# MircoWerner/VkRadixSort

Measured on AMD Instinct MI355X. Metric: Gkeys/s sorting 10^8 uint32 at 1/2/4/8 MI355X; % of HBM roofline, higher is better.
Workload: dtype u32

## Files before the change

vkradixsort_amd/csrc/vrs_local_sort.hpp:

```cpp
#pragma once
#include "vrs_device.hpp"

namespace vrs {

constexpr int kLeanRow = 512 + 64;
constexpr int kLeanMaxVec = 7;
template <bool STREAM>
__device__ __forceinline__ void store_sorted(uint4 *p, const uint4 &q) {
    if constexpr (STREAM) {
        typedef uint32_t u32x4 __attribute__((ext_vector_type(4)));
        const u32x4 v = {q.x, q.y, q.z, q.w};
        __builtin_nontemporal_store(v, reinterpret_cast<u32x4 *>(p));
    } else {
        *p = q;
    }
}

template <int STRIDE, int VEC>
__device__ __forceinline__ void load_rows(uint32_t (&k)[4 * VEC], const uint32_t *src, uint32_t words, uint32_t t) {
    const uint32_t nvec = (words + 3u) / 4u;
#pragma unroll
    for (int j = 0; j < VEC; ++j) {
        uint32_t v = j * STRIDE + t;
        if (j == VEC - 1) v = v < nvec ? v : nvec - 1u;
        const uint4 q = reinterpret_cast<const uint4 *>(src)[v];
        k[4 * j] = q.x;
        k[4 * j + 1] = q.y;
        k[4 * j + 2] = q.z;
        k[4 * j + 3] = q.w;
    }
}

template <int THREADS, int VEC, bool GUARD, bool STREAM = false, bool ALIGNED_IN = false>
__device__ __forceinline__ void lean_sort_body(uint32_t (&k)[4 * VEC], uint32_t *abase, uint32_t mis, uint32_t n, uint32_t *s_keys,
                                               uint32_t *s_hist2, uint32_t *s_tmp, bool guard1, bool guard2, uint32_t mis_in) {
    constexpr int WAVES = THREADS / 64, ITEMS = 4 * VEC, PER = 512 / THREADS;
    const uint32_t tid = threadIdx.x, lane = tid & 63u, wave = tid >> 6;
    const uint32_t end = mis + n;
    const uint32_t nvec = (end + 3u) / 4u;
    uint32_t rank[ITEMS];
    uint32_t *s_hist = s_hist2 + WAVES * kLeanRow;
#pragma unroll
    for (int j = 0; j < VEC; ++j)
#pragma unroll
        for (int c = 0; c < 4; ++c) {
            uint32_t a = (k[4 * j + c] << 2) & 0x7FCu;
            if (ALIGNED_IN ? j >= VEC - 2 : (j == 0 || j == VEC - 1)) {
                const uint32_t q = 4u * (j * THREADS + tid) + c;
                a = (q - mis_in < n) ? a : 2048u + 4u * lane;
            }
            uint32_t *counter = reinterpret_cast<uint32_t *>(reinterpret_cast<char *>(s_hist) + a);
            if (GUARD && guard1) {
                const uint32_t a0 = __builtin_amdgcn_readfirstlane(a);
                if (__ballot(a == a0) == ~0ull) {
                    uint32_t old = 0;
                    if (lane == 0u) old = __hip_atomic_fetch_add(counter, 256u, __ATOMIC_RELAXED, __HIP_MEMORY_SCOPE_WORKGROUP);
                    rank[4 * j + c] = __builtin_amdgcn_readfirstlane(old) + 4u * lane;
                    continue;
                }
            }
            rank[4 * j + c] = __hip_atomic_fetch_add(counter, 4u, __ATOMIC_RELAXED, __HIP_MEMORY_SCOPE_WORKGROUP);
        }
    __syncthreads();
    {
        uint32_t c[PER], total = 0;
        if constexpr (PER == 2) {
            const uint2 q = reinterpret_cast<const uint2 *>(s_hist)[tid];
            c[0] = q.x;
            c[1] = q.y;
            total = q.x + q.y;
        } else {
            c[0] = s_hist[tid];
            total = c[0];
        }
        uint32_t incl = total;
#pragma unroll
        for (int o = 1; o < 64; o <<= 1) {
            const uint32_t t = __shfl_up(incl, o);
            if (lane >= static_cast<uint32_t>(o)) incl += t;
        }
        if (lane == 63u) s_tmp[wave] = incl;
        __syncthreads();
        uint32_t acc = incl - total;
#pragma unroll
        for (int v = 0; v < WAVES; ++v) acc += (static_cast<uint32_t>(v) < wave) ? s_tmp[v] : 0u;
        if constexpr (PER == 2) reinterpret_cast<uint2 *>(s_hist)[tid] = make_uint2(acc, acc + c[0]);
        else s_hist[tid] = acc;
    }
    __syncthreads();
#pragma unroll
    for (int j = 0; j < VEC; ++j)
#pragma unroll
        for (int c = 0; c < 4; ++c) {
            uint32_t a = (opaque(k[4 * j + c]) << 2) & 0x7FCu;
            if (ALIGNED_IN ? j >= VEC - 2 : (j == 0 || j == VEC - 1)) {
                const uint32_t q = 4u * (j * THREADS + tid) + c;
                const bool valid = q - mis_in < n;
                a = valid ? a : 2048u + 4u * lane;
                const uint32_t r = rank[4 * j + c] + *reinterpret_cast<const uint32_t *>(reinterpret_cast<const char *>(s_hist) + a);
                rank[4 * j + c] = valid ? r : 4u * (q < mis_in ? n + q : q);
                continue;
            }
            rank[4 * j + c] += *reinterpret_cast<const uint32_t *>(reinterpret_cast<const char *>(s_hist) + a);
        }
#pragma unroll
    for (int i = 0; i < ITEMS; ++i) {
        const uint32_t Lb = rank[i];
        const uint32_t ph = (Lb & ~1023u) | ((Lb & 252u) << 2) | ((Lb >> 6) & 12u);
        *reinterpret_cast<uint32_t *>(reinterpret_cast<char *>(s_keys) + ph) = k[i];
    }
    __syncthreads();
    const uint32_t seg = wave * (ITEMS * 64);
#pragma unroll
    for (int g = 0; g < VEC; ++g) {
        const uint4 t = reinterpret_cast<const uint4 *>(s_keys + seg + g * 256)[lane];
        k[4 * g] = t.x;
        k[4 * g + 1] = t.y;
        k[4 * g + 2] = t.z;
        k[4 * g + 3] = t.w;
    }
    char *my = reinterpret_cast<char *>(s_hist2 + wave * kLeanRow);
    constexpr int kEmptyItems = (4 * THREADS + 3 + 63) / 64;
    constexpr int kFirstMaybeEmpty = ITEMS >= kEmptyItems ? ITEMS - kEmptyItems : 0;
#pragma unroll
    for (int i = 0; i < ITEMS; ++i) {
        uint32_t a = (k[i] >> 7) & 0x7FCu;
        if (i >= kFirstMaybeEmpty) a = (seg + i * 64 + lane < n) ? a : 2048u + 4u * lane;
        uint32_t *counter = reinterpret_cast<uint32_t *>(my + a);
        if (GUARD && guard2) {
            const uint32_t a0 = __builtin_amdgcn_readfirstlane(a);
            if (__ballot(a == a0) == ~0ull) {
                uint32_t old = 0;
                if (lane == 0u) old = __hip_atomic_fetch_add(counter, 256u, __ATOMIC_RELAXED, __HIP_MEMORY_SCOPE_WORKGROUP);
                rank[i] = __builtin_amdgcn_readfirstlane(old) + 4u * lane;
                continue;
            }
        }
        rank[i] = __hip_atomic_fetch_add(counter, 4u, __ATOMIC_RELAXED, __HIP_MEMORY_SCOPE_WORKGROUP);
    }
    __syncthreads();
    {
        uint32_t c[WAVES][PER], total = 0;
#pragma unroll
        for (int v = 0; v < WAVES; ++v) {
            if constexpr (PER == 2) {
                const uint2 q = reinterpret_cast<const uint2 *>(s_hist2 + v * kLeanRow)[tid];
                c[v][0] = q.x;
                c[v][1] = q.y;
                total += q.x + q.y;
            } else {
                c[v][0] = s_hist2[v * kLeanRow + tid];
                total += c[v][0];
            }
        }
        uint32_t incl = total;
#pragma unroll
        for (int o = 1; o < 64; o <<= 1) {
            const uint32_t t = __shfl_up(incl, o);
            if (lane >= static_cast<uint32_t>(o)) incl += t;
        }
        if (lane == 63u) s_tmp[wave] = incl;
        __syncthreads();
        uint32_t acc = incl - total + 4u * mis;
#pragma unroll
        for (int v = 0; v < WAVES; ++v) acc += (static_cast<uint32_t>(v) < wave) ? s_tmp[v] : 0u;
        uint32_t out[WAVES][PER];
#pragma unroll
        for (int p_ = 0; p_ < PER; ++p_)
#pragma unroll
            for (int v = 0; v < WAVES; ++v) {
                out[v][p_] = acc;
                acc += c[v][p_];
            }
#pragma unroll
        for (int v = 0; v < WAVES; ++v) {
            if constexpr (PER == 2) reinterpret_cast<uint2 *>(s_hist2 + v * kLeanRow)[tid] = make_uint2(out[v][0], out[v][1]);
            else s_hist2[v * kLeanRow + tid] = out[v][0];
        }
    }
    __syncthreads();
#pragma unroll
    for (int i = 0; i < ITEMS; ++i) {
        uint32_t a = (opaque(k[i]) >> 7) & 0x7FCu;
        if (i >= kFirstMaybeEmpty) {
            const uint32_t L = seg + i * 64 + lane;
            a = L < n ? a : 2048u + 4u * lane;
            const uint32_t r = rank[i] + *reinterpret_cast<const uint32_t *>(my + a);
            rank[i] = L < n ? r : 4u * (mis + L);
            continue;
        }
        rank[i] += *reinterpret_cast<const uint32_t *>(my + a);
    }
#pragma unroll
    for (int i = 0; i < ITEMS; ++i) *reinterpret_cast<uint32_t *>(reinterpret_cast<char *>(s_keys) + rank[i]) = k[i];
    __syncthreads();
#pragma unroll
    for (int j = 0; j < VEC; ++j) {
        const uint32_t v = j * THREADS + tid;
        if (j > 0 && j < VEC - 1) {
            store_sorted<STREAM>(reinterpret_cast<uint4 *>(abase) + v, reinterpret_cast<const uint4 *>(s_keys)[v]);
        } else if (v < nvec) {
            const uint4 q4 = reinterpret_cast<const uint4 *>(s_keys)[v];
            const uint32_t q = 4u * v;
            if (q >= mis && q + 4u <= end) {
                store_sorted<STREAM>(reinterpret_cast<uint4 *>(abase) + v, q4);
            } else {
                if (q + 0u - mis < n) abase[q + 0u] = q4.x;
                if (q + 1u - mis < n) abase[q + 1u] = q4.y;
                if (q + 2u - mis < n) abase[q + 2u] = q4.z;
                if (q + 3u - mis < n) abase[q + 3u] = q4.w;
            }
        }
    }
}

__device__ __forceinline__ void wave_phase() {
    __builtin_amdgcn_fence(__ATOMIC_RELEASE, "wavefront");
    __builtin_amdgcn_wave_barrier();
    __builtin_amdgcn_fence(__ATOMIC_ACQUIRE, "wavefront");
}
__device__ __forceinline__ void wave_scan512(uint32_t *tbl, uint32_t lane, uint32_t start) {
    uint4 a = reinterpret_cast<uint4 *>(tbl)[2 * lane], b = reinterpret_cast<uint4 *>(tbl)[2 * lane + 1];
    const uint32_t s = a.x + a.y + a.z + a.w + b.x + b.y + b.z + b.w;
    uint32_t incl = s;
#pragma unroll
    for (int o = 1; o < 64; o <<= 1) {
        const uint32_t t = __shfl_up(incl, o);
        if (lane >= static_cast<uint32_t>(o)) incl += t;
    }
    uint32_t acc = incl - s + start;
    uint4 oa, ob;
    oa.x = acc; acc += a.x; oa.y = acc; acc += a.y; oa.z = acc; acc += a.z; oa.w = acc; acc += a.w;
    ob.x = acc; acc += b.x; ob.y = acc; acc += b.y; ob.z = acc; acc += b.z; ob.w = acc;
    reinterpret_cast<uint4 *>(tbl)[2 * lane] = oa;
    reinterpret_cast<uint4 *>(tbl)[2 * lane + 1] = ob;
}
template <int VEC, bool GUARD, bool STREAM = false, bool ALIGNED_IN = false>
__device__ __forceinline__ void wave_sort_body(uint32_t (&k)[4 * VEC], uint32_t *abase, uint32_t mis, uint32_t n, uint32_t *s_keys,
                                               uint32_t *tbl, bool guard1, bool guard2, uint32_t mis_in) {
    constexpr int ITEMS = 4 * VEC;
    const uint32_t lane = threadIdx.x & 63u;
    const uint32_t end = mis + n, nvec = (end + 3u) / 4u;
    uint32_t rank[ITEMS];
    char *tb = reinterpret_cast<char *>(tbl);
    const auto zero_table = [&] {
        reinterpret_cast<uint4 *>(tbl)[2 * lane] = make_uint4(0, 0, 0, 0);
        reinterpret_cast<uint4 *>(tbl)[2 * lane + 1] = make_uint4(0, 0, 0, 0);
        if (lane < 16u) reinterpret_cast<uint4 *>(tbl)[128 + lane] = make_uint4(0, 0, 0, 0);
    };
    const auto ranked_add = [&](uint32_t a, bool guard) -> uint32_t {
        uint32_t *counter = reinterpret_cast<uint32_t *>(tb + a);
        if (GUARD && guard) {
            const uint32_t a0 = __builtin_amdgcn_readfirstlane(a);
            if (__ballot(a == a0) == ~0ull) {
                uint32_t old = 0;
                if (lane == 0u) old = __hip_atomic_fetch_add(counter, 256u, __ATOMIC_RELAXED, __HIP_MEMORY_SCOPE_WORKGROUP);
                return __builtin_amdgcn_readfirstlane(old) + 4u * lane;
            }
        }
        return __hip_atomic_fetch_add(counter, 4u, __ATOMIC_RELAXED, __HIP_MEMORY_SCOPE_WORKGROUP);
    };
#pragma unroll
    for (int i = 0; i < ITEMS; ++i) {
        uint32_t a = (k[i] << 2) & 0x7FCu;
        if (ALIGNED_IN ? i >= ITEMS - 8 : (i < 4 || i >= ITEMS - 4)) {
            const uint32_t q = 4u * ((i >> 2) * 64 + lane) + (i & 3);
            a = (q - mis_in < n) ? a : 2048u + 4u * lane;
        }
        rank[i] = ranked_add(a, guard1);
    }
    wave_phase();
    wave_scan512(tbl, lane, 0u);
    wave_phase();
#pragma unroll
    for (int i = 0; i < ITEMS; ++i) {
        uint32_t a = (opaque(k[i]) << 2) & 0x7FCu;
        if (ALIGNED_IN ? i >= ITEMS - 8 : (i < 4 || i >= ITEMS - 4)) {
            const uint32_t q = 4u * ((i >> 2) * 64 + lane) + (i & 3);
            const bool valid = q - mis_in < n;
            a = valid ? a : 2048u + 4u * lane;
            const uint32_t r = rank[i] + *reinterpret_cast<const uint32_t *>(tb + a);
            rank[i] = valid ? r : 4u * (q < mis_in ? n + q : q);
            continue;
        }
        rank[i] += *reinterpret_cast<const uint32_t *>(tb + a);
    }
#pragma unroll
    for (int i = 0; i < ITEMS; ++i) {
        const uint32_t Lb = rank[i];
        const uint32_t ph = (Lb & ~1023u) | ((Lb & 252u) << 2) | ((Lb >> 6) & 12u);
        *reinterpret_cast<uint32_t *>(reinterpret_cast<char *>(s_keys) + ph) = k[i];
    }
    wave_phase();
    zero_table();
#pragma unroll
    for (int g = 0; g < VEC; ++g) {
        const uint4 t = reinterpret_cast<const uint4 *>(s_keys + g * 256)[lane];
        k[4 * g] = t.x;
        k[4 * g + 1] = t.y;
        k[4 * g + 2] = t.z;
        k[4 * g + 3] = t.w;
    }
    wave_phase();
#pragma unroll
    for (int i = 0; i < ITEMS; ++i) {
        uint32_t a = (k[i] >> 7) & 0x7FCu;
        a = (i * 64 + lane < n) ? a : 2048u + 4u * lane;
        rank[i] = ranked_add(a, guard2);
    }
    wave_phase();
    wave_scan512(tbl, lane, 4u * mis);
    wave_phase();
#pragma unroll
    for (int i = 0; i < ITEMS; ++i) {
        const uint32_t L = i * 64 + lane;
        uint32_t a = (opaque(k[i]) >> 7) & 0x7FCu;
        a = L < n ? a : 2048u + 4u * lane;
        const uint32_t r = rank[i] + *reinterpret_cast<const uint32_t *>(tb + a);
        rank[i] = L < n ? r : 4u * (mis + L);
    }
#pragma unroll
    for (int i = 0; i < ITEMS; ++i) *reinterpret_cast<uint32_t *>(reinterpret_cast<char *>(s_keys) + rank[i]) = k[i];
    wave_phase();
#pragma unroll
    for (int j = 0; j < VEC; ++j) {
        const uint32_t v = j * 64 + lane;
        if (v < nvec) {
            const uint4 q4 = reinterpret_cast<const uint4 *>(s_keys)[v];
            const uint32_t q = 4u * v;
            if (q >= mis && q + 4u <= end) {
                store_sorted<STREAM>(reinterpret_cast<uint4 *>(abase) + v, q4);
            } else {
                if (q + 0u - mis < n) abase[q + 0u] = q4.x;
                if (q + 1u - mis < n) abase[q + 1u] = q4.y;
                if (q + 2u - mis < n) abase[q + 2u] = q4.z;
                if (q + 3u - mis < n) abase[q + 3u] = q4.w;
            }
        }
    }
}

struct NoHook {
    __device__ __forceinline__ void operator()() const {}
};
template <int THREADS, int ITEMS, int BITS, bool PAIRS, bool STABLE, typename K = uint32_t, typename Hook = NoHook>
__device__ __forceinline__ void local_pass(K (&key)[ITEMS], uint32_t (&val)[PAIRS ? ITEMS : 1], K *s_keys,
                                           uint32_t *s_vals, uint32_t *s_hist, uint32_t *s_tmp, uint32_t shift, uint32_t n, Hook scanned = Hook()) {
    constexpr int WAVES = THREADS / 64, BINS = 1 << BITS, TABLES = STABLE ? WAVES : 1, PER = BINS >= THREADS ? BINS / THREADS : 1;
    static_assert(PER * THREADS == BINS || (PER == 1 && THREADS % BINS == 0), "every scanning thread owns PER whole bins");
    const uint32_t tid = threadIdx.x, lane = tid & 63u, wave = tid >> 6;
    const bool scans = THREADS <= BINS || tid < static_cast<uint32_t>(BINS);
    for (uint32_t c = tid; c < TABLES * BINS; c += THREADS) s_hist[c] = 0;
    __syncthreads();
    uint32_t *my = s_hist + (STABLE ? wave * BINS : 0u);
    const uint32_t seg = wave * (ITEMS * 64) + lane;
    uint32_t rank[ITEMS];
#pragma unroll
    for (int i = 0; i < ITEMS; ++i) {
        rank[i] = seg + i * 64;
        if (rank[i] < n) {
            const uint32_t d = static_cast<uint32_t>(key[i] >> shift) & (BINS - 1);
            const uint32_t d0 = __builtin_amdgcn_readfirstlane(d);
            const uint64_t active = __ballot(1);
            if (__ballot(d == d0) == active) {
                uint32_t old = 0;
                if (__builtin_amdgcn_mbcnt_hi(static_cast<uint32_t>(active >> 32), __builtin_amdgcn_mbcnt_lo(static_cast<uint32_t>(active), 0u)) == 0u)
                    old = __hip_atomic_fetch_add(&my[d0], static_cast<uint32_t>(__popcll(active)), __ATOMIC_RELAXED, __HIP_MEMORY_SCOPE_WORKGROUP);
                rank[i] = __builtin_amdgcn_readfirstlane(old) +
                          __builtin_amdgcn_mbcnt_hi(static_cast<uint32_t>(active >> 32), __builtin_amdgcn_mbcnt_lo(static_cast<uint32_t>(active), 0u));
            } else {
                rank[i] = __hip_atomic_fetch_add(&my[d], 1u, __ATOMIC_RELAXED, __HIP_MEMORY_SCOPE_WORKGROUP);
            }
        }
    }
    __syncthreads();
    {
        uint32_t c[TABLES][PER], total = 0;
#pragma unroll
        for (int v = 0; v < TABLES; ++v) {
            if constexpr (PER == 2) {
                const uint2 q = reinterpret_cast<const uint2 *>(s_hist + v * BINS)[tid];
                c[v][0] = q.x;
                c[v][1] = q.y;
                total += q.x + q.y;
            } else {
#pragma unroll
                for (int p_ = 0; p_ < PER; ++p_) {
                    c[v][p_] = scans ? s_hist[v * BINS + tid * PER + p_] : 0u;
                    total += c[v][p_];
                }
            }
        }
        uint32_t incl = total;
#pragma unroll
        for (int o = 1; o < 64; o <<= 1) {
            const uint32_t t = __shfl_up(incl, o);
            if (lane >= static_cast<uint32_t>(o)) incl += t;
        }
        if (lane == 63u) s_tmp[wave] = incl;
        __syncthreads();
        uint32_t acc = incl - total;
#pragma unroll
        for (int v = 0; v < WAVES; ++v) acc += (static_cast<uint32_t>(v) < wave) ? s_tmp[v] : 0u;
        uint32_t out[TABLES][PER];
#pragma unroll
        for (int p_ = 0; p_ < PER; ++p_) {
#pragma unroll
            for (int v = 0; v < TABLES; ++v) {
                out[v][p_] = acc;
                acc += c[v][p_];
            }
        }
#pragma unroll
        for (int v = 0; v < TABLES; ++v) {
            if constexpr (PER == 2) {
                reinterpret_cast<uint2 *>(s_hist + v * BINS)[tid] = make_uint2(out[v][0], out[v][1]);
            } else {
#pragma unroll
                for (int p_ = 0; p_ < PER; ++p_)
                    if (scans) s_hist[v * BINS + tid * PER + p_] = out[v][p_];
            }
        }
    }
    __syncthreads();
    scanned();
#pragma unroll
    for (int i = 0; i < ITEMS; ++i)
        if (seg + i * 64 < n) rank[i] += my[static_cast<uint32_t>(key[i] >> shift) & (BINS - 1)];
#pragma unroll
    for (int i = 0; i < ITEMS; ++i)
        if (seg + i * 64 < n) s_keys[rank[i]] = key[i];
    if constexpr (PAIRS) {
#pragma unroll
        for (int i = 0; i < ITEMS; ++i)
            if (seg + i * 64 < n) s_vals[rank[i]] = val[i];
    }
    __syncthreads();
#pragma unroll
    for (int i = 0; i < ITEMS; ++i) key[i] = s_keys[seg + i * 64];
    if constexpr (PAIRS) {
#pragma unroll
        for (int i = 0; i < ITEMS; ++i) val[i] = s_vals[seg + i * 64];
    }
    __syncthreads();
}

template <int THREADS, int ITEMS, bool PAIRS, bool STREAM = false>
__device__ __forceinline__ void local_sort_bucket_to(const uint32_t *src, const uint32_t *src_vals, uint32_t *bucket, uint32_t *bucket_vals, uint32_t n,
                                                     uint32_t *s_keys, uint32_t *s_vals, uint32_t *s_hist, uint32_t *s_tmp) {
    constexpr int BITS = 9;
    const uint32_t lane = threadIdx.x & 63u, wave = threadIdx.x >> 6;
// ... 100 lines not shown
```

vkradixsort_amd/csrc/vrs_msd_hybrid.hip:

```cpp
#include "vrs_device.hpp"
#include "vrs_local_sort.hpp"
#include "vrs_plan.hpp"

#include <algorithm>
#include <type_traits>

namespace vrs {

constexpr int kLocalThreads = 256, kLocalItems = 26;
constexpr uint32_t kLocalCap = kLocalThreads * kLocalItems;


__global__ __launch_bounds__(1024) void msd_count_u64_kernel(const uint64_t *__restrict__ keys, uint32_t n, uint32_t group_len,
                                                            uint32_t slices, uint4 *__restrict__ status, uint32_t status_vecs,
                                                            uint32_t *__restrict__ msd_hist, uint32_t *__restrict__ msd_slices) {
    constexpr uint32_t THREADS = 1024, UNROLL = 4;
    __shared__ uint32_t s_msd[kMsdBuckets];
    __shared__ unsigned long long s_or;
    const uint32_t tid = threadIdx.x, lane = tid & 63u;
    if (tid == 0) s_or = 0;
    for (uint32_t c = tid; c < kMsdBuckets; c += THREADS) s_msd[c] = 0;
    {
        const uint4 zero = make_uint4(0, 0, 0, 0);
        const uint32_t per = (status_vecs + gridDim.x - 1) / gridDim.x;
// ... 265 lines not shown
            __syncthreads();
            recount_keys(cnt, keys_in + first, done, dg);
            __syncthreads();
            if (threadIdx.x < kBins) lb.recounted = cnt[threadIdx.x];
            __syncthreads();
        }
        lb.col = status + (static_cast<size_t>(pt[k]) * 8u + x) * kBins + (threadIdx.x & 255u);
        lb.stride = static_cast<size_t>(8) * kBins;
        lb.index = static_cast<int>(i);
        lb.tag = 6u << kLbTagShift;
        lb.budget = spin_budget;
        lb.seed = threadIdx.x < (1u << sub_bits) ? msd->base[(a << sub_bits) + threadIdx.x] : 0u;
        if (valid == kTile)
            scatter_chunk<K, ITEMS, 8, PAIRS, RANK, true>(sm, keys_in + begin, vin, keys_out, values_out, valid, dg, unused, lb, NoPieces{}, stream_in);
        else
            scatter_chunk<K, ITEMS, 8, PAIRS, RANK, false>(sm, keys_in + begin, vin, keys_out, values_out, valid, dg, unused, lb);
    }
}

__device__ __forceinline__ uint32_t local_sort_bucket_of_block() {
    return gridDim.x - 1u - blockIdx.x;
}

__device__ __forceinline__ void rearm_reservation(uint32_t *__restrict__ cursors, uint32_t threads) {
    constexpr uint32_t kRowsA = 2u * kStreams;
    uint32_t *cursor_b = cursors + kRowsA * 256u, *back_b = cursor_b + kMsdBuckets;
    const uint32_t b = blockIdx.x;
    if (threadIdx.x == 0) {
        cursor_b[b] = 0;
        back_b[b] = 0;
    }
    if (b < kRowsA)
        for (uint32_t c = threadIdx.x; c < 256u; c += threads) cursors[b * 256u + c] = 0;
}

template <int THREADS, int VEC>
__device__ __attribute__((noinline)) void lean_sort_guarded(uint32_t *abase, uint32_t mis, uint32_t n, uint32_t *s_keys, uint32_t *s_hist2,
                                                           uint32_t *s_tmp, uint32_t guards);

template <int THREADS, int VEC>
__device__ __forceinline__ void lean_sort_bucket(uint32_t *abase, uint32_t mis, uint32_t n, uint32_t *s_keys, uint32_t *s_hist2,
                                                 uint32_t *s_tmp) {
    constexpr int WAVES = THREADS / 64, ITEMS = 4 * VEC;
    static_assert(THREADS == 256 || THREADS == 512, "the scans give every thread 2 or 1 bins");
    const uint32_t tid = threadIdx.x, lane = tid & 63u, wave = tid >> 6;
    const uint32_t end = mis + n;
    const uint32_t nvec = (end + 3u) / 4u;
    uint32_t k[ITEMS];
#pragma unroll
    for (int j = 0; j < VEC; ++j) {
        uint32_t v = j * THREADS + tid;
        if (j == VEC - 1) v = v < nvec ? v : nvec - 1u;
        const uint4 t = reinterpret_cast<const uint4 *>(abase)[v];
        k[4 * j] = t.x;
        k[4 * j + 1] = t.y;
        k[4 * j + 2] = t.z;
        k[4 * j + 3] = t.w;
    }
    uint32_t *s_hist = s_hist2 + WAVES * kLeanRow;
    {
        constexpr uint32_t kVecs = (WAVES + 1) * kLeanRow / 4;
        for (uint32_t c = tid; c < kVecs; c += THREADS) reinterpret_cast<uint4 *>(s_hist2)[c] = make_uint4(0, 0, 0, 0);
    }
    {
        uint32_t skew = 0;
#pragma unroll
        for (int c = 0; c < 4; ++c) {
            const uint32_t a1 = k[c] & 511u, a2 = (k[c] >> 9) & 511u;
            skew |= __popcll(__ballot(a1 == __builtin_amdgcn_readfirstlane(a1))) >= 32 ? 1u : 0u;
            skew |= __popcll(__ballot(a2 == __builtin_amdgcn_readfirstlane(a2))) >= 32 ? 2u : 0u;
        }
        if (lane == 0u) s_tmp[16 + wave] = skew;
    }
    __syncthreads();
    uint32_t guards = 0;
#pragma unroll
    for (int v = 0; v < WAVES; ++v) guards |= s_tmp[16 + v];
    guards = __builtin_amdgcn_readfirstlane(guards);
    if (guards == 0u) lean_sort_body<THREADS, VEC, false>(k, abase, mis, n, s_keys, s_hist2, s_tmp, false, false, mis);
    else lean_sort_guarded<THREADS, VEC>(abase, mis, n, s_keys, s_hist2, s_tmp, guards);
}

template <int THREADS, int VEC>
__device__ __attribute__((noinline)) void lean_sort_guarded(uint32_t *abase, uint32_t mis, uint32_t n, uint32_t *s_keys, uint32_t *s_hist2,
                                                           uint32_t *s_tmp, uint32_t guards) {
    constexpr int ITEMS = 4 * VEC;
    const uint32_t nvec = (mis + n + 3u) / 4u;
    uint32_t k[ITEMS];
#pragma unroll
    for (int j = 0; j < VEC; ++j) {
        uint32_t v = j * THREADS + threadIdx.x;
        if (j == VEC - 1) v = v < nvec ? v : nvec - 1u;
        const uint4 t = reinterpret_cast<const uint4 *>(abase)[v];
        k[4 * j] = t.x;
        k[4 * j + 1] = t.y;
        k[4 * j + 2] = t.z;
        k[4 * j + 3] = t.w;
    }
    lean_sort_body<THREADS, VEC, true>(k, abase, mis, n, s_keys, s_hist2, s_tmp, (guards & 1u) != 0u, (guards & 2u) != 0u, mis);
}

template <int THREADS>
__global__ __launch_bounds__(THREADS, 4) void msd_local_sort_keys_kernel(uint32_t *__restrict__ keys, const MsdPlan *__restrict__ msd, StatusClear sc,
                                                                         uint32_t *__restrict__ cursors) {
    __shared__ __attribute__((aligned(16))) uint32_t s_keys[THREADS * 4 * kLeanMaxVec + 4];
    __shared__ __attribute__((aligned(16))) uint32_t s_hist[(THREADS / 64 + 1) * kLeanRow];
    __shared__ uint32_t s_tmp[32];
    if (msd->ok == 0u) return;
    rearm_reservation(cursors, THREADS);
    clear_status_share(sc, THREADS);
    const uint32_t bkt = local_sort_bucket_of_block();
    const uint32_t begin = msd->base[bkt], n = msd->base[bkt + 1] - begin;
    const uint32_t mis = static_cast<uint32_t>((reinterpret_cast<uintptr_t>(keys + begin) >> 2) & 3u);
    if (n == 0 || mis + n > THREADS * 4u * kLeanMaxVec) return;
    uint32_t *abase = keys + begin - mis;
    switch ((mis + n + 4u * THREADS - 1u) / (4u * THREADS)) {
        case 1: lean_sort_bucket<THREADS, 1>(abase, mis, n, s_keys, s_hist, s_tmp); break;
        case 2: lean_sort_bucket<THREADS, 2>(abase, mis, n, s_keys, s_hist, s_tmp); break;
        case 3: lean_sort_bucket<THREADS, 3>(abase, mis, n, s_keys, s_hist, s_tmp); break;
        case 4: lean_sort_bucket<THREADS, 4>(abase, mis, n, s_keys, s_hist, s_tmp); break;
        case 5: lean_sort_bucket<THREADS, 5>(abase, mis, n, s_keys, s_hist, s_tmp); break;
        case 6: lean_sort_bucket<THREADS, 6>(abase, mis, n, s_keys, s_hist, s_tmp); break;
        default: lean_sort_bucket<THREADS, 7>(abase, mis, n, s_keys, s_hist, s_tmp); break;
    }
}
constexpr uint32_t kLeanCap = 256u * 4u * kLeanMaxVec - 3u, kLeanBigCap = 512u * 4u * kLeanMaxVec - 3u;


template <int VEC>
__device__ __attribute__((noinline)) void wave_sort_guarded(uint32_t *abase, uint32_t mis, uint32_t n, uint32_t *s_keys, uint32_t *tbl,
                                                           uint32_t skew);

template <int VEC>
__device__ __forceinline__ void wave_sort_bucket(uint32_t *abase, uint32_t mis, uint32_t n, uint32_t *s_keys, uint32_t *tbl) {
    constexpr int ITEMS = 4 * VEC;
    const uint32_t lane = threadIdx.x & 63u;
    const uint32_t end = mis + n, nvec = (end + 3u) / 4u;
    uint32_t k[ITEMS];
#pragma unroll
    for (int j = 0; j < VEC; ++j) {
        uint32_t v = j * 64 + lane;
        if (j == VEC - 1) v = v < nvec ? v : nvec - 1u;
        const uint4 t = reinterpret_cast<const uint4 *>(abase)[v];
        k[4 * j] = t.x;
        k[4 * j + 1] = t.y;
        k[4 * j + 2] = t.z;
        k[4 * j + 3] = t.w;
    }
    char *tb = reinterpret_cast<char *>(tbl);
    const auto zero_table = [&] {
        reinterpret_cast<uint4 *>(tbl)[2 * lane] = make_uint4(0, 0, 0, 0);
        reinterpret_cast<uint4 *>(tbl)[2 * lane + 1] = make_uint4(0, 0, 0, 0);
        if (lane < 16u) reinterpret_cast<uint4 *>(tbl)[128 + lane] = make_uint4(0, 0, 0, 0);
    };
    zero_table();
    uint32_t skew = 0;
#pragma unroll
    for (int c = 0; c < 4; ++c) {
        const uint32_t a1 = k[c] & 511u, a2 = (k[c] >> 9) & 511u;
        skew |= __popcll(__ballot(a1 == __builtin_amdgcn_readfirstlane(a1))) >= 32 ? 1u : 0u;
        skew |= __popcll(__ballot(a2 == __builtin_amdgcn_readfirstlane(a2))) >= 32 ? 2u : 0u;
    }
    skew = __builtin_amdgcn_readfirstlane(skew);
    wave_phase();
    if (skew == 0u) wave_sort_body<VEC, false>(k, abase, mis, n, s_keys, tbl, false, false, mis);
    else wave_sort_guarded<VEC>(abase, mis, n, s_keys, tbl, skew);
}

template <int VEC>
__device__ __attribute__((noinline)) void wave_sort_guarded(uint32_t *abase, uint32_t mis, uint32_t n, uint32_t *s_keys, uint32_t *tbl,
                                                           uint32_t skew) {
    constexpr int ITEMS = 4 * VEC;
    const uint32_t lane = threadIdx.x & 63u;
    const uint32_t nvec = (mis + n + 3u) / 4u;
    uint32_t k[ITEMS];
#pragma unroll
    for (int j = 0; j < VEC; ++j) {
        uint32_t v = j * 64 + lane;
        if (j == VEC - 1) v = v < nvec ? v : nvec - 1u;
        const uint4 t = reinterpret_cast<const uint4 *>(abase)[v];
        k[4 * j] = t.x;
        k[4 * j + 1] = t.y;
        k[4 * j + 2] = t.z;
        k[4 * j + 3] = t.w;
    }
    wave_sort_body<VEC, true>(k, abase, mis, n, s_keys, tbl, (skew & 1u) != 0u, (skew & 2u) != 0u, mis);
}

constexpr uint32_t kWaveCap = 64u * 4u * kLeanMaxVec - 3u;
__global__ __launch_bounds__(64, 4) void msd_local_sort_wave_kernel(uint32_t *__restrict__ keys, const MsdPlan *__restrict__ msd, StatusClear sc,
                                                                  uint32_t *__restrict__ cursors) {
    __shared__ __attribute__((aligned(16))) uint32_t s_keys[64 * 4 * kLeanMaxVec + 4];
    __shared__ __attribute__((aligned(16))) uint32_t s_tbl[kLeanRow];
    if (msd->ok == 0u) return;
    rearm_reservation(cursors, 64);
    clear_status_share(sc, 64);
    const uint32_t bkt = local_sort_bucket_of_block();
    const uint32_t begin = msd->base[bkt], n = msd->base[bkt + 1] - begin;
    const uint32_t mis = static_cast<uint32_t>((reinterpret_cast<uintptr_t>(keys + begin) >> 2) & 3u);
    if (n == 0 || mis + n > 64u * 4u * kLeanMaxVec) return;
    uint32_t *abase = keys + begin - mis;
    switch ((mis + n + 255u) / 256u) {
        case 1: wave_sort_bucket<1>(abase, mis, n, s_keys, s_tbl); break;
        case 2: wave_sort_bucket<2>(abase, mis, n, s_keys, s_tbl); break;
        case 3: wave_sort_bucket<3>(abase, mis, n, s_keys, s_tbl); break;
        case 4: wave_sort_bucket<4>(abase, mis, n, s_keys, s_tbl); break;
        case 5: wave_sort_bucket<5>(abase, mis, n, s_keys, s_tbl); break;
        case 6: wave_sort_bucket<6>(abase, mis, n, s_keys, s_tbl); break;
        default: wave_sort_bucket<7>(abase, mis, n, s_keys, s_tbl); break;
    }
}

constexpr int kLocalPairThreads = 512, kLocalPairItems = kLocalCap / kLocalPairThreads;
constexpr int kLocalPairThreadsBig = 1024;
constexpr uint32_t kLocalCapBig = kLocalPairThreadsBig * kLocalPairItems;
template <int THREADS>
__global__ __launch_bounds__(THREADS, 4) void msd_local_sort_pairs_kernel(uint32_t *__restrict__ keys,
                                                                                         uint32_t *__restrict__ values,
                                                                                         const MsdPlan *__restrict__ msd, StatusClear sc,
// ... 272 lines not shown
```

vkradixsort_amd/csrc/vrs_msd_pool_local.hip:

```cpp
#include "vrs_local_sort.hpp"

#include <cstdlib>


namespace vrs {

namespace {

template <int THREADS, int VEC>
__device__ __attribute__((noinline)) void slack_sort_guarded(const uint32_t *src, uint32_t *abase, uint32_t mis, uint32_t n, uint32_t *s_keys,
                                                            uint32_t *s_hist2, uint32_t *s_tmp, uint32_t guards) {
    uint32_t k[4 * VEC];
    load_rows<THREADS, VEC>(k, src, n, threadIdx.x);
    lean_sort_body<THREADS, VEC, true, true, true>(k, abase, mis, n, s_keys, s_hist2, s_tmp, (guards & 1u) != 0u, (guards & 2u) != 0u, 0u);
}

template <int THREADS, int VEC>
__device__ __forceinline__ void slack_sort_bucket(const uint32_t *src, uint32_t *abase, uint32_t mis, uint32_t n, uint32_t *s_keys, uint32_t *s_hist2,
                                                  uint32_t *s_tmp) {
    constexpr int WAVES = THREADS / 64;
    const uint32_t tid = threadIdx.x, lane = tid & 63u, wave = tid >> 6;
    uint32_t k[4 * VEC];
    load_rows<THREADS, VEC>(k, src, n, threadIdx.x);
    {
        constexpr uint32_t kVecs = (WAVES + 1) * kLeanRow / 4;
        for (uint32_t c = tid; c < kVecs; c += THREADS) reinterpret_cast<uint4 *>(s_hist2)[c] = make_uint4(0, 0, 0, 0);
    }
    {
        uint32_t skew = 0;
#pragma unroll
        for (int c = 0; c < 4; ++c) {
            const uint32_t a1 = k[c] & 511u, a2 = (k[c] >> 9) & 511u;
            skew |= __popcll(__ballot(a1 == __builtin_amdgcn_readfirstlane(a1))) >= 32 ? 1u : 0u;
            skew |= __popcll(__ballot(a2 == __builtin_amdgcn_readfirstlane(a2))) >= 32 ? 2u : 0u;
        }
        if (lane == 0u) s_tmp[16 + wave] = skew;
    }
    __syncthreads();
    uint32_t guards = 0;
#pragma unroll
    for (int v = 0; v < WAVES; ++v) guards |= s_tmp[16 + v];
    guards = __builtin_amdgcn_readfirstlane(guards);
    if (guards == 0u) lean_sort_body<THREADS, VEC, false, true, true>(k, abase, mis, n, s_keys, s_hist2, s_tmp, false, false, 0u);
    else slack_sort_guarded<THREADS, VEC>(src, abase, mis, n, s_keys, s_hist2, s_tmp, guards);
}

template <int THREADS, uint32_t CAPACITY, uint32_t SUBBITS>
__device__ __forceinline__ bool pool_bucket(const uint32_t *__restrict__ slack, uint32_t *__restrict__ keys_out, MsdPlan *__restrict__ msd,
                                            const PoolPlan *__restrict__ pool, uint32_t *__restrict__ cursors, OnesweepPlanHead *__restrict__ dev_head,
                                            OnesweepPlanHead *host_head, uint32_t stamp, uint32_t *host_log, uint32_t retry, uint32_t par,
                                            const uint32_t *&src, uint32_t *&abase, uint32_t &mis, uint32_t &n, const StatusClear sc = {nullptr, 0u}) {
    constexpr uint32_t SUB = 1u << SUBBITS, PER = SUB / 64u;
    const uint32_t b = gridDim.x - 1u - blockIdx.x, a = b >> SUBBITS, c = b & (SUB - 1u);
    const uint32_t lane = threadIdx.x & 63u;
    uint32_t cnt[PER];
#pragma unroll
    for (uint32_t q = 0; q < PER; ++q) cnt[q] = pool->sub_cursor[(a << SUBBITS) + 64u * q + lane];
    const uint32_t start = pool->sub_start[b], top = pool->top_base[a];
    const uint32_t flags = pool->fail[par], mx = pool->max_bucket;
    const uint32_t ok = (pool->ok_a != 0u && (flags & (retry ? 1u : 3u)) == 0u && (retry == 0u || mx <= CAPACITY - 3u)) ? 1u : 0u;
    const uint32_t again = (ok == 0u && retry == 0u && pool->ok_a != 0u && flags == 2u) ? mx : 0u;
    if (blockIdx.x == 0 && threadIdx.x == 0) {
        msd->ok = ok;
        dev_head->msd_ok = ok;
        dev_head->msd_max_bucket = again;
        dev_head->lsd_missing = 1u;
        if (host_head) {
            __hip_atomic_store(&host_head->lsd_missing, 1u, __ATOMIC_RELAXED, __HIP_MEMORY_SCOPE_SYSTEM);
            __hip_atomic_store(&host_head->msd_ok, ok, __ATOMIC_RELAXED, __HIP_MEMORY_SCOPE_SYSTEM);
            __hip_atomic_store(&host_head->msd_max_bucket, again, __ATOMIC_RELAXED, __HIP_MEMORY_SCOPE_SYSTEM);
            if (host_log) __hip_atomic_store(&host_log[stamp & (kMsdLogWords - 1u)], (stamp << 1) | ok, __ATOMIC_RELAXED, __HIP_MEMORY_SCOPE_SYSTEM);
            __threadfence_system();
            __hip_atomic_store(&host_head->ready, stamp, __ATOMIC_RELEASE, __HIP_MEMORY_SCOPE_SYSTEM);
        }
    }
    if (ok == 0u) return false;
    clear_status_share(sc, THREADS);
    if (blockIdx.x < 2u * kStreams)
        for (uint32_t q = threadIdx.x; q < 256u; q += THREADS) cursors[blockIdx.x * 256u + q] = 0;
    uint32_t before = 0;
    n = 0;
#pragma unroll
    for (uint32_t q = 0; q < PER; ++q) {
        before += 64u * q + lane < c ? cnt[q] : 0u;
        const uint32_t v = __builtin_amdgcn_readlane(cnt[q], c & 63u);
        n = (c >> 6) == q ? v : n;
    }
#pragma unroll
    for (int o = 32; o >= 1; o >>= 1) before += __shfl_xor(before, o);
    const uint32_t begin = top + __builtin_amdgcn_readfirstlane(before);
    mis = static_cast<uint32_t>((reinterpret_cast<uintptr_t>(keys_out + begin) >> 2) & 3u);
    if (n == 0 || mis + n > CAPACITY) return false;
    abase = keys_out + begin - mis;
    src = slack + start;
    return true;
}

template <int THREADS, int MAXVEC, int WGS, uint32_t SUBBITS>
__global__ __launch_bounds__(THREADS, WGS *(THREADS / 64) / 4) void pool_local_sort_kernel(const uint32_t *__restrict__ slack, uint32_t *__restrict__ keys_out,
                                                                                          MsdPlan *__restrict__ msd, const PoolPlan *__restrict__ pool,
                                                                                          uint32_t *__restrict__ cursors, OnesweepPlanHead *__restrict__ dev_head,
                                                                                          OnesweepPlanHead *host_head, uint32_t stamp, uint32_t *host_log, uint32_t retry, uint32_t par) {
    __shared__ __attribute__((aligned(16))) uint32_t s_keys[THREADS * 4 * MAXVEC + 4];
    __shared__ __attribute__((aligned(16))) uint32_t s_hist[(THREADS / 64 + 1) * kLeanRow];
    __shared__ uint32_t s_tmp[32];
    const uint32_t *src;
    uint32_t *abase, mis, n;
    if (!pool_bucket<THREADS, THREADS * 4u * MAXVEC, SUBBITS>(slack, keys_out, msd, pool, cursors, dev_head, host_head, stamp, host_log, retry, par, src, abase, mis, n)) return;
    const uint32_t rows = (mis + n + 4u * THREADS - 1u) / (4u * THREADS);
    if constexpr (MAXVEC == 4) {
        switch (rows) {
            case 1: slack_sort_bucket<THREADS, 1>(src, abase, mis, n, s_keys, s_hist, s_tmp); break;
            case 2: slack_sort_bucket<THREADS, 2>(src, abase, mis, n, s_keys, s_hist, s_tmp); break;
            case 3: slack_sort_bucket<THREADS, 3>(src, abase, mis, n, s_keys, s_hist, s_tmp); break;
            default: slack_sort_bucket<THREADS, 4>(src, abase, mis, n, s_keys, s_hist, s_tmp); break;
        }
    } else {
        switch (rows) {
            case 1: slack_sort_bucket<THREADS, 1>(src, abase, mis, n, s_keys, s_hist, s_tmp); break;
            case 2: slack_sort_bucket<THREADS, 2>(src, abase, mis, n, s_keys, s_hist, s_tmp); break;
            case 3: slack_sort_bucket<THREADS, 3>(src, abase, mis, n, s_keys, s_hist, s_tmp); break;
            case 4: slack_sort_bucket<THREADS, 4>(src, abase, mis, n, s_keys, s_hist, s_tmp); break;
            case 5: slack_sort_bucket<THREADS, 5>(src, abase, mis, n, s_keys, s_hist, s_tmp); break;
            case 6: slack_sort_bucket<THREADS, 6>(src, abase, mis, n, s_keys, s_hist, s_tmp); break;
            default: slack_sort_bucket<THREADS, 7>(src, abase, mis, n, s_keys, s_hist, s_tmp); break;
        }
    }
}

template <int THREADS, uint32_t SUBBITS, bool PACKED>
__global__ __launch_bounds__(THREADS, (PACKED && THREADS == 512) ? 6 : 4) void pool_local_sort_pairs_kernel(const uint32_t *__restrict__ slack, uint32_t *__restrict__ keys_out,
                                                                          MsdPlan *__restrict__ msd, const PoolPlan *__restrict__ pool,
                                                                          uint32_t *__restrict__ cursors, OnesweepPlanHead *__restrict__ dev_head,
                                                                          OnesweepPlanHead *host_head, uint32_t stamp, uint32_t *host_log, uint32_t retry,
                                                                          uint32_t par, PoolPayloads pv) {
    constexpr int WAVES = THREADS / 64;
    constexpr uint32_t CAP = THREADS * kPoolPairItems;
    __shared__ uint32_t s_keys[CAP];
    __shared__ uint32_t s_vals[PACKED ? 1 : CAP];
    __shared__ uint32_t s_hist[WAVES << 9];
    __shared__ uint32_t s_tmp[1 + WAVES];
    const uint32_t *src;
    uint32_t *abase, mis, n;
    const StatusClear sc{reinterpret_cast<uint4 *>(pv.status), static_cast<uint32_t>(pv.status_words / 4u)};
    if (!pool_bucket<THREADS, CAP + 3u, SUBBITS>(slack, keys_out, msd, pool, cursors, dev_head, host_head, stamp, host_log, retry, par, src, abase, mis, n, sc)) return;
    if (n > CAP) return;
    uint32_t *bucket = abase + mis, *bvals = pv.values_home + (bucket - keys_out);
    const uint32_t *svals = pv.slack_values + (src - slack);
    const uint32_t used = (n + THREADS - 1u) / THREADS;
    const uint32_t lowbits = pool->shift + kMsdBits - pv.top_bits - SUBBITS;
    constexpr int IDXB = THREADS == 512 ? 13 : 14;
    if constexpr (PACKED) {
        if (lowbits > 18u) return;
        if (used <= 4) local_sort_packed_pairs_to<THREADS, 4, IDXB, true>(src, svals, bucket, bvals, n, lowbits, s_keys, s_hist, s_tmp);
        else if (used <= 8) local_sort_packed_pairs_to<THREADS, 8, IDXB, true>(src, svals, bucket, bvals, n, lowbits, s_keys, s_hist, s_tmp);
        else if (used <= 10) local_sort_packed_pairs_to<THREADS, 10, IDXB, true>(src, svals, bucket, bvals, n, lowbits, s_keys, s_hist, s_tmp);
        else if (used <= 12) local_sort_packed_pairs_to<THREADS, 12, IDXB, true>(src, svals, bucket, bvals, n, lowbits, s_keys, s_hist, s_tmp);
        else local_sort_packed_pairs_to<THREADS, kPoolPairItems, IDXB, true>(src, svals, bucket, bvals, n, lowbits, s_keys, s_hist, s_tmp);
// ... 122 lines not shown
```

Measured before the change: 199.3.

## Use DPP wave scans, vectorized LDS reads and scheduling pins in local sorts

```diff
diff --git a/vkradixsort_amd/csrc/vrs_local_sort.hpp b/vkradixsort_amd/csrc/vrs_local_sort.hpp
--- a/vkradixsort_amd/csrc/vrs_local_sort.hpp
+++ b/vkradixsort_amd/csrc/vrs_local_sort.hpp
@@ -16,6 +16,7 @@
     }
 }
 
+__device__ __forceinline__ void rows_in_order() { __builtin_amdgcn_sched_barrier(0); }
 template <int STRIDE, int VEC>
 __device__ __forceinline__ void load_rows(uint32_t (&k)[4 * VEC], const uint32_t *src, uint32_t words, uint32_t t) {
     const uint32_t nvec = (words + 3u) / 4u;
@@ -24,11 +25,41 @@
         uint32_t v = j * STRIDE + t;
         if (j == VEC - 1) v = v < nvec ? v : nvec - 1u;
         const uint4 q = reinterpret_cast<const uint4 *>(src)[v];
+        if (j + 1 < VEC) rows_in_order();
         k[4 * j] = q.x;
         k[4 * j + 1] = q.y;
         k[4 * j + 2] = q.z;
         k[4 * j + 3] = q.w;
     }
+}
+
+__device__ __forceinline__ uint32_t wave_inclusive_sum(uint32_t x) {
+    x += __builtin_amdgcn_update_dpp(0u, x, 0x111, 0xf, 0xf, false);
+    x += __builtin_amdgcn_update_dpp(0u, x, 0x112, 0xf, 0xf, false);
+    x += __builtin_amdgcn_update_dpp(0u, x, 0x114, 0xf, 0xf, false);
+    x += __builtin_amdgcn_update_dpp(0u, x, 0x118, 0xf, 0xf, false);
+    x += __builtin_amdgcn_update_dpp(0u, x, 0x142, 0xa, 0xf, false);
+    x += __builtin_amdgcn_update_dpp(0u, x, 0x143, 0xc, 0xf, false);
+    return x;
+}
+
+__device__ __forceinline__ void pinned(uint32_t &x) { asm volatile("" : "+v"(x)); }
+
+template <int WAVES>
+__device__ __forceinline__ uint32_t waves_before(const uint32_t *s_tmp, uint32_t wave) {
+    static_assert(WAVES % 4 == 0, "whole 16-byte vectors");
+    uint4 t[WAVES / 4];
+#pragma unroll
+    for (int g = 0; g < WAVES / 4; ++g) t[g] = reinterpret_cast<const uint4 *>(s_tmp)[g];
+    uint32_t sum = 0;
+#pragma unroll
+    for (int g = 0; g < WAVES / 4; ++g) {
+        sum += (4u * g + 0u < wave) ? t[g].x : 0u;
+        sum += (4u * g + 1u < wave) ? t[g].y : 0u;
+        sum += (4u * g + 2u < wave) ? t[g].z : 0u;
+        sum += (4u * g + 3u < wave) ? t[g].w : 0u;
+    }
+    return sum;
 }
 
 template <int THREADS, int VEC, bool GUARD, bool STREAM = false, bool ALIGNED_IN = false>
@@ -73,17 +104,10 @@
             c[0] = s_hist[tid];
             total = c[0];
         }
-        uint32_t incl = total;
-#pragma unroll
-        for (int o = 1; o < 64; o <<= 1) {
-            const uint32_t t = __shfl_up(incl, o);
-            if (lane >= static_cast<uint32_t>(o)) incl += t;
-        }
+        const uint32_t incl = wave_inclusive_sum(total);
         if (lane == 63u) s_tmp[wave] = incl;
         __syncthreads();
-        uint32_t acc = incl - total;
-#pragma unroll
-        for (int v = 0; v < WAVES; ++v) acc += (static_cast<uint32_t>(v) < wave) ? s_tmp[v] : 0u;
+        uint32_t acc = incl - total + waves_before<WAVES>(s_tmp, wave);
         if constexpr (PER == 2) reinterpret_cast<uint2 *>(s_hist)[tid] = make_uint2(acc, acc + c[0]);
         else s_hist[tid] = acc;
     }
@@ -95,13 +119,24 @@
             uint32_t a = (opaque(k[4 * j + c]) << 2) & 0x7FCu;
             if (ALIGNED_IN ? j >= VEC - 2 : (j == 0 || j == VEC - 1)) {
                 const uint32_t q = 4u * (j * THREADS + tid) + c;
-                const bool valid = q - mis_in < n;
-                a = valid ? a : 2048u + 4u * lane;
-                const uint32_t r = rank[4 * j + c] + *reinterpret_cast<const uint32_t *>(reinterpret_cast<const char *>(s_hist) + a);
-                rank[4 * j + c] = valid ? r : 4u * (q < mis_in ? n + q : q);
-                continue;
+                a = (q - mis_in < n) ? a : 2048u + 4u * lane;
             }
             rank[4 * j + c] += *reinterpret_cast<const uint32_t *>(reinterpret_cast<const char *>(s_hist) + a);
+        }
+#pragma unroll
+    for (int j = 0; j < VEC; ++j)
+        if (ALIGNED_IN ? j >= VEC - 2 : (j == 0 || j == VEC - 1)) {
+#pragma unroll
+            for (int c = 0; c < 4; ++c) pinned(rank[4 * j + c]);
+        }
+#pragma unroll
+    for (int j = 0; j < VEC; ++j)
+        if (ALIGNED_IN ? j >= VEC - 2 : (j == 0 || j == VEC - 1)) {
+#pragma unroll
+            for (int c = 0; c < 4; ++c) {
+                const uint32_t q = 4u * (j * THREADS + tid) + c;
+                rank[4 * j + c] = (q - mis_in < n) ? rank[4 * j + c] : 4u * (q < mis_in ? n + q : q);
+            }
         }
 #pragma unroll
     for (int i = 0; i < ITEMS; ++i) {
@@ -153,17 +188,10 @@
                 total += c[v][0];
             }
         }
-        uint32_t incl = total;
-#pragma unroll
-        for (int o = 1; o < 64; o <<= 1) {
-            const uint32_t t = __shfl_up(incl, o);
-            if (lane >= static_cast<uint32_t>(o)) incl += t;
-        }
+        const uint32_t incl = wave_inclusive_sum(total);
         if (lane == 63u) s_tmp[wave] = incl;
         __syncthreads();
-        uint32_t acc = incl - total + 4u * mis;
-#pragma unroll
-        for (int v = 0; v < WAVES; ++v) acc += (static_cast<uint32_t>(v) < wave) ? s_tmp[v] : 0u;
+        uint32_t acc = incl - total + 4u * mis + waves_before<WAVES>(s_tmp, wave);
         uint32_t out[WAVES][PER];
 #pragma unroll
         for (int p_ = 0; p_ < PER; ++p_)
@@ -182,21 +210,23 @@
 #pragma unroll
     for (int i = 0; i < ITEMS; ++i) {
         uint32_t a = (opaque(k[i]) >> 7) & 0x7FCu;
-        if (i >= kFirstMaybeEmpty) {
-            const uint32_t L = seg + i * 64 + lane;
-            a = L < n ? a : 2048u + 4u * lane;
-            const uint32_t r = rank[i] + *reinterpret_cast<const uint32_t *>(my + a);
-            rank[i] = L < n ? r : 4u * (mis + L);
-            continue;
-        }
+        if (i >= kFirstMaybeEmpty) a = (seg + i * 64 + lane < n) ? a : 2048u + 4u * lane;
         rank[i] += *reinterpret_cast<const uint32_t *>(my + a);
     }
 #pragma unroll
+    for (int i = kFirstMaybeEmpty; i < ITEMS; ++i) pinned(rank[i]);
+#pragma unroll
+    for (int i = kFirstMaybeEmpty; i < ITEMS; ++i) {
+        const uint32_t L = seg + i * 64 + lane;
+        rank[i] = L < n ? rank[i] : 4u * (mis + L);
+    }
+#pragma unroll
     for (int i = 0; i < ITEMS; ++i) *reinterpret_cast<uint32_t *>(reinterpret_cast<char *>(s_keys) + rank[i]) = k[i];
     __syncthreads();
+    const uint32_t ts = ALIGNED_IN ? tid : opaque(tid);
 #pragma unroll
     for (int j = 0; j < VEC; ++j) {
-        const uint32_t v = j * THREADS + tid;
+        const uint32_t v = j * THREADS + ts;
         if (j > 0 && j < VEC - 1) {
             store_sorted<STREAM>(reinterpret_cast<uint4 *>(abase) + v, reinterpret_cast<const uint4 *>(s_keys)[v]);
         } else if (v < nvec) {
@@ -222,13 +252,7 @@
 __device__ __forceinline__ void wave_scan512(uint32_t *tbl, uint32_t lane, uint32_t start) {
     uint4 a = reinterpret_cast<uint4 *>(tbl)[2 * lane], b = reinterpret_cast<uint4 *>(tbl)[2 * lane + 1];
     const uint32_t s = a.x + a.y + a.z + a.w + b.x + b.y + b.z + b.w;
-    uint32_t incl = s;
-#pragma unroll
-    for (int o = 1; o < 64; o <<= 1) {
-        const uint32_t t = __shfl_up(incl, o);
-        if (lane >= static_cast<uint32_t>(o)) incl += t;
-    }
-    uint32_t acc = incl - s + start;
+    uint32_t acc = wave_inclusive_sum(s) - s + start;
     uint4 oa, ob;
     oa.x = acc; acc += a.x; oa.y = acc; acc += a.y; oa.z = acc; acc += a.z; oa.w = acc; acc += a.w;
     ob.x = acc; acc += b.x; ob.y = acc; acc += b.y; ob.z = acc; acc += b.z; ob.w = acc;
@@ -277,14 +301,19 @@
         uint32_t a = (opaque(k[i]) << 2) & 0x7FCu;
         if (ALIGNED_IN ? i >= ITEMS - 8 : (i < 4 || i >= ITEMS - 4)) {
             const uint32_t q = 4u * ((i >> 2) * 64 + lane) + (i & 3);
-            const bool valid = q - mis_in < n;
-            a = valid ? a : 2048u + 4u * lane;
-            const uint32_t r = rank[i] + *reinterpret_cast<const uint32_t *>(tb + a);
-            rank[i] = valid ? r : 4u * (q < mis_in ? n + q : q);
-            continue;
+            a = (q - mis_in < n) ? a : 2048u + 4u * lane;
         }
         rank[i] += *reinterpret_cast<const uint32_t *>(tb + a);
     }
+#pragma unroll
+    for (int i = 0; i < ITEMS; ++i)
+        if (ALIGNED_IN ? i >= ITEMS - 8 : (i < 4 || i >= ITEMS - 4)) pinned(rank[i]);
+#pragma unroll
+    for (int i = 0; i < ITEMS; ++i)
+        if (ALIGNED_IN ? i >= ITEMS - 8 : (i < 4 || i >= ITEMS - 4)) {
+            const uint32_t q = 4u * ((i >> 2) * 64 + lane) + (i & 3);
+            rank[i] = (q - mis_in < n) ? rank[i] : 4u * (q < mis_in ? n + q : q);
+        }
 #pragma unroll
     for (int i = 0; i < ITEMS; ++i) {
         const uint32_t Lb = rank[i];
@@ -313,18 +342,24 @@
     wave_phase();
 #pragma unroll
     for (int i = 0; i < ITEMS; ++i) {
+        uint32_t a = (opaque(k[i]) >> 7) & 0x7FCu;
+        a = (i * 64 + lane < n) ? a : 2048u + 4u * lane;
+        rank[i] += *reinterpret_cast<const uint32_t *>(tb + a);
+    }
+#pragma unroll
+    for (int i = 0; i < ITEMS; ++i) pinned(rank[i]);
+#pragma unroll
+    for (int i = 0; i < ITEMS; ++i) {
         const uint32_t L = i * 64 + lane;
-        uint32_t a = (opaque(k[i]) >> 7) & 0x7FCu;
-        a = L < n ? a : 2048u + 4u * lane;
-        const uint32_t r = rank[i] + *reinterpret_cast<const uint32_t *>(tb + a);
-        rank[i] = L < n ? r : 4u * (mis + L);
+        rank[i] = L < n ? rank[i] : 4u * (mis + L);
     }
 #pragma unroll
     for (int i = 0; i < ITEMS; ++i) *reinterpret_cast<uint32_t *>(reinterpret_cast<char *>(s_keys) + rank[i]) = k[i];
     wave_phase();
+    const uint32_t ls = ALIGNED_IN ? lane : opaque(lane);
 #pragma unroll
     for (int j = 0; j < VEC; ++j) {
-        const uint32_t v = j * 64 + lane;
+        const uint32_t v = j * 64 + ls;
         if (v < nvec) {
             const uint4 q4 = reinterpret_cast<const uint4 *>(s_keys)[v];
             const uint32_t q = 4u * v;
@@ -391,12 +426,7 @@
                 }
             }
         }
-        uint32_t incl = total;
-#pragma unroll
-        for (int o = 1; o < 64; o <<= 1) {
-            const uint32_t t = __shfl_up(incl, o);
-            if (lane >= static_cast<uint32_t>(o)) incl += t;
-        }
+        const uint32_t incl = wave_inclusive_sum(total);
         if (lane == 63u) s_tmp[wave] = incl;
         __syncthreads();
         uint32_t acc = incl - total;
diff --git a/vkradixsort_amd/csrc/vrs_msd_hybrid.hip b/vkradixsort_amd/csrc/vrs_msd_hybrid.hip
--- a/vkradixsort_amd/csrc/vrs_msd_hybrid.hip
+++ b/vkradixsort_amd/csrc/vrs_msd_hybrid.hip
@@ -341,6 +341,7 @@
         uint32_t v = j * THREADS + tid;
         if (j == VEC - 1) v = v < nvec ? v : nvec - 1u;
         const uint4 t = reinterpret_cast<const uint4 *>(abase)[v];
+        if (j + 1 < VEC) rows_in_order();
         k[4 * j] = t.x;
         k[4 * j + 1] = t.y;
         k[4 * j + 2] = t.z;
@@ -364,7 +365,10 @@
     __syncthreads();
     uint32_t guards = 0;
 #pragma unroll
-    for (int v = 0; v < WAVES; ++v) guards |= s_tmp[16 + v];
+    for (int g = 0; g < WAVES / 4; ++g) {
+        const uint4 t = reinterpret_cast<const uint4 *>(s_tmp + 16)[g];
+        guards |= t.x | t.y | t.z | t.w;
+    }
     guards = __builtin_amdgcn_readfirstlane(guards);
     if (guards == 0u) lean_sort_body<THREADS, VEC, false>(k, abase, mis, n, s_keys, s_hist2, s_tmp, false, false, mis);
     else lean_sort_guarded<THREADS, VEC>(abase, mis, n, s_keys, s_hist2, s_tmp, guards);
@@ -394,7 +398,7 @@
                                                                          uint32_t *__restrict__ cursors) {
     __shared__ __attribute__((aligned(16))) uint32_t s_keys[THREADS * 4 * kLeanMaxVec + 4];
     __shared__ __attribute__((aligned(16))) uint32_t s_hist[(THREADS / 64 + 1) * kLeanRow];
-    __shared__ uint32_t s_tmp[32];
+    __shared__ __attribute__((aligned(16))) uint32_t s_tmp[32];
     if (msd->ok == 0u) return;
     rearm_reservation(cursors, THREADS);
     clear_status_share(sc, THREADS);
@@ -453,7 +457,11 @@
     skew = __builtin_amdgcn_readfirstlane(skew);
     wave_phase();
     if (skew == 0u) wave_sort_body<VEC, false>(k, abase, mis, n, s_keys, tbl, false, false, mis);
-    else wave_sort_guarded<VEC>(abase, mis, n, s_keys, tbl, skew);
+    else {
+        uint32_t *table = tbl;
+        asm volatile("" : "+v"(table));
+        wave_sort_guarded<VEC>(abase, mis, n, s_keys, table, skew);
+    }
 }
 
 template <int VEC>
diff --git a/vkradixsort_amd/csrc/vrs_msd_pool_local.hip b/vkradixsort_amd/csrc/vrs_msd_pool_local.hip
--- a/vkradixsort_amd/csrc/vrs_msd_pool_local.hip
+++ b/vkradixsort_amd/csrc/vrs_msd_pool_local.hip
@@ -39,7 +39,10 @@
     __syncthreads();
     uint32_t guards = 0;
 #pragma unroll
-    for (int v = 0; v < WAVES; ++v) guards |= s_tmp[16 + v];
+    for (int g = 0; g < WAVES / 4; ++g) {
+        const uint4 t = reinterpret_cast<const uint4 *>(s_tmp + 16)[g];
+        guards |= t.x | t.y | t.z | t.w;
+    }
     guards = __builtin_amdgcn_readfirstlane(guards);
     if (guards == 0u) lean_sort_body<THREADS, VEC, false, true, true>(k, abase, mis, n, s_keys, s_hist2, s_tmp, false, false, 0u);
     else slack_sort_guarded<THREADS, VEC>(src, abase, mis, n, s_keys, s_hist2, s_tmp, guards);
@@ -103,7 +106,7 @@
                                                                                           OnesweepPlanHead *host_head, uint32_t stamp, uint32_t *host_log, uint32_t retry, uint32_t par) {
     __shared__ __attribute__((aligned(16))) uint32_t s_keys[THREADS * 4 * MAXVEC + 4];
     __shared__ __attribute__((aligned(16))) uint32_t s_hist[(THREADS / 64 + 1) * kLeanRow];
-    __shared__ uint32_t s_tmp[32];
+    __shared__ __attribute__((aligned(16))) uint32_t s_tmp[32];
     const uint32_t *src;
     uint32_t *abase, mis, n;
     if (!pool_bucket<THREADS, THREADS * 4u * MAXVEC, SUBBITS>(slack, keys_out, msd, pool, cursors, dev_head, host_head, stamp, host_log, retry, par, src, abase, mis, n)) return;
```

Result: faster. 203.6, median of 6 (+2.1%).
